# jeuneS2/csolve

Measured on AMD Instinct MI355X. Metric: constraint propagations/sec + nodes/sec, queens-N, 1/2/4/8 MI355X, higher is better.
Workload: dtype int32

## Files before the change

csolve_amd/csrc/cs_capi.hip:

```cpp
#include <hip/hip_runtime.h>
#include <chrono>

#include <dlfcn.h>
#include <stdarg.h>
#include <stdio.h>
#include <stdlib.h>
#include <string.h>

#include <mutex>

#include "../../include/csolve_gpu.h"
#include "cs_kernels.hip.h"
#include "cs_shave.hip.h"
#include "cs_step.hip.h"
#include "cs_dive.hip.h"
#include "cs_walk.hip.h"
#include "cs_chain.hip.h"
#include "cs_internal.h"

static thread_local char g_err[512] = "";

static int set_err(int code, const char *fmt, ...) {
  va_list ap;
  va_start(ap, fmt);
// ... 884 lines not shown
  if ((rc = lds_limit((size_t)h->n_vars * sizeof(cs_val) + 16, (const void *)cs_eval_root))) return rc;
  if ((rc = lds_limit((size_t)h->n_vars * sizeof(cs_val) + 16, (const void *)cs_eval_clauses))) return rc;
  if ((rc = plan_kernel(&m->plan.traced, (const void *)cs_propagate_events<true, false, true>, m->slice * CS_WAVES_PER_BLOCK,
                        CS_WAVES_PER_BLOCK)))
    return rc;
  const int per = (m->img->n_clauses + CS_WAVE - 1) / CS_WAVE;
  m->plan.rounds_cpl = m->img->n_clauses <= 0 || per > 8 ? 0 : (per <= 1 ? 1 : (per <= 2 ? 2 : (per <= 4 ? 4 : 8)));
  if (m->plan.rounds_cpl) {
#define CS_PICK6(CPL)                                                                              \
  m->plan.rounds.fn = m->has_tree_adj ? (const void *)cs_propagate_clause_rounds<CPL, true>         \
                                      : (const void *)cs_propagate_clause_rounds<CPL, false>
    switch (m->plan.rounds_cpl) {
    case 1: CS_PICK6(1); break;
    case 2: CS_PICK6(2); break;
    case 4: CS_PICK6(4); break;
    default: CS_PICK6(8); break;
    }
#undef CS_PICK6
    m->plan.rounds.lds = ((((size_t)h->n_vars * sizeof(cs_val) + 16 + 15) & ~(size_t)15)) * CS_WAVES_PER_BLOCK;
    m->plan.rounds.waves = CS_WAVES_PER_BLOCK;
    m->plan.rounds.per_cu = 8;
    if (m->plan.rounds.lds <= CS_CU_LDS) {
      for (int family = 0; family < WALK_FAMILIES; family++) {
        cs_planned *k = &m->plan.walk[family];
        if ((rc = plan_kernel(k, walk_kernel(family, m->plan.rounds_cpl, m->has_tree_adj), m->plan.rounds.lds, CS_WAVES_PER_BLOCK)))
          return rc;
        int occ = 0;
        if (hipOccupancyMaxActiveBlocksPerMultiprocessor(&occ, k->fn, CS_BLOCK, k->lds) == hipSuccess && occ >= 1 && occ < k->per_cu)
          k->per_cu = occ;
        if (k->per_cu < 1) k->per_cu = 1;
      }
      if ((rc = upload(h->dom, (size_t)h->n_vars * sizeof(cs_val), (int **)&m->d_walk_root))) return rc;
    }
  }
  m->plan.max_width = 2;
  for (int32_t v = 0; v < h->n_vars; v++) {
    const int64_t w = (int64_t)h->dom[v].hi - (int64_t)h->dom[v].lo + 1;
    if (w > m->plan.max_width) m->plan.max_width = w > 0x7fffffff ? 0x7fffffff : (int)w;
  }
  return CSGPU_OK;
}

static int plan_lds_resident(csgpu_model *m) {
  const cs_model *h = m->host;
  if (m->img->packed_width == 0) return CSGPU_OK;
  const size_t off_bytes = (((size_t)h->n_vars * 2 * sizeof(int)) + 15) & ~(size_t)15;
  const size_t adj_bytes = (((size_t)m->img->n_adj * (size_t)m->img->packed_width) + 15) & ~(size_t)15;
  const size_t lds_slice = ((size_t)h->n_vars * sizeof(cs_val) + (2 * (size_t)m->tab.n_words + 1) * sizeof(unsigned) + 15) & ~(size_t)15;
  m->lds_adj_global = 0;
  int waves_max = 16, waves = 0;
  size_t bytes = 0;
  { const char *e = getenv("CSGPU_K2_WAVES"); if (e != NULL && atoi(e) >= 4 && atoi(e) <= 16) waves_max = atoi(e); }
  for (int w = waves_max; w >= 4; w--) {
    const size_t need = off_bytes + adj_bytes + (size_t)w * lds_slice;
    if (need <= CS_CU_LDS) {
      waves = w;
      bytes = need;
      break;
    }
  }
  const char *force = getenv("CSGPU_K2_ADJ");
  const int want_global = force != NULL && force[0] == 'g';
  if (want_global && 8 * lds_slice <= CS_CU_LDS) {
    m->lds_adj_global = 1;
    waves = 8;
    bytes = 8 * lds_slice;
  }
  { const char *e = getenv("CSGPU_K2_CSZ"); m->k2_csz = e != NULL && atoi(e) >= 1 && atoi(e) <= CS_CHUNK ? atoi(e) : 0; }
  if (!waves) return CSGPU_OK;
  int rc;
  if ((rc = upload(m->img->adj_packed, (size_t)m->img->n_adj * (size_t)m->img->packed_width, (int **)&m->d_adj_packed)))
    return rc;
  if ((rc = plan_kernel(&m->plan.lds, ne_lds_kernel(m->img->packed_width, h->n_vars, m->lds_adj_global), bytes, waves)))
    return rc;
  if (m->plan.lds.per_cu < 1) m->plan.lds.per_cu = 1;
  return CSGPU_OK;
}

static int64_t widest_root_domain(const csgpu_model *m) {
  const cs_model *h = m->host;
  int64_t width = 1;
  for (int32_t v = 0; v < h->n_vars; v++) {
    const int64_t w = (int64_t)h->dom[v].hi - (int64_t)h->dom[v].lo + 1;
    if (w > width) width = w;
  }
  return width;
}

static int forbidden_sets_shape(const csgpu_model *m, int *fw_out, size_t *lds_out) {
  const cs_model *h = m->host;
  if (m->img->sym_width == 0 || m->not_root) return 0;
  const int64_t width = widest_root_domain(m);
  const int fw = width <= 64 ? 1 : (width <= 128 ? 2 : (width <= 256 ? 4 : 0));
  if (!fw) return 0;
  const size_t n_words = ((size_t)h->n_vars + 31) / 32;
  const size_t off_bytes = (((size_t)h->n_vars * 2 * sizeof(int)) + 15) & ~(size_t)15;
  const size_t base_bytes = (((size_t)h->n_vars * sizeof(int)) + 15) & ~(size_t)15;
  const size_t adj_bytes = (((size_t)m->img->sym_n_adj * (size_t)m->img->sym_width) + 15) & ~(size_t)15;
  const size_t sl = ((size_t)h->n_vars * sizeof(cs_val) + (size_t)h->n_vars * fw * 8 + (2 * n_words + 2) * sizeof(unsigned) + 15) &
                    ~(size_t)15;
  int waves = 16;
  for (; waves >= 1; waves--)
    if (off_bytes + base_bytes + adj_bytes + (size_t)waves * sl <= CS_CU_LDS) break;
  if (waves < 1) return 0;
  *fw_out = fw;
  *lds_out = off_bytes + base_bytes + adj_bytes + (size_t)waves * sl;
  return waves;
}

static int plan_forbidden_sets(csgpu_model *m) {
  const cs_model *h = m->host;
  int fw = 0;
  size_t lds = 0;
  const int waves = forbidden_sets_shape(m, &fw, &lds);
  if (!waves) return CSGPU_OK;
  m->fb_words = fw;
  int *lo = (int *)malloc((size_t)(h->n_vars ? h->n_vars : 1) * sizeof(int));
  for (int32_t v = 0; v < h->n_vars; v++) lo[v] = h->dom[v].lo;
  int rc = upload(lo, (size_t)h->n_vars * sizeof(int), &m->d_root_lo);
  free(lo);
  if (rc) return rc;
  if ((rc = upload(m->img->sym_off, ((size_t)h->n_vars + 1) * sizeof(int), &m->d_sym_off))) return rc;
  if ((rc = upload(m->img->sym_packed, (size_t)m->img->sym_n_adj * (size_t)m->img->sym_width, (int **)&m->d_sym_packed)))
    return rc;
  if ((rc = plan_kernel(&m->plan.bitset, ne_bitset_kernel(m->img->sym_width, fw, h->n_vars), lds, waves))) return rc;
  if (m->plan.bitset.per_cu < 1) m->plan.bitset.per_cu = 1;
  return CSGPU_OK;
}

static int dense_table_waves(const csgpu_model *m, size_t *bytes_out) {
  if (m->img->dense_width == 0) return 0;
  const size_t bytes = (size_t)m->host->n_vars * m->img->dense_slots * m->img->dense_cols * m->img->dense_width;
  int best = 0, waves = 0;
  for (int w = 4; w <= 16; w <<= 1)
    if (resident_per_cu(bytes, w) * w > best) { best = resident_per_cu(bytes, w) * w; waves = w; }
  *bytes_out = bytes;
  return waves;
}

static int plan_dense_table(csgpu_model *m) {
  const cs_model *h = m->host;
  if (!m->fb_words) return CSGPU_OK;
  const int n = h->n_vars, width = m->img->dense_width, slots = m->img->dense_slots;
  size_t bytes = 0;
  const int waves = dense_table_waves(m, &bytes);
  if (!waves) return CSGPU_OK;
  m->dense_bytes = bytes;
  int rc;
  if ((rc = upload(m->img->dense_tab, bytes, (int **)&m->d_dense_tab))) return rc;
  for (int variant = 0; variant < 4; variant++)
    if ((rc = plan_kernel(&m->plan.regs[variant], ne_regs_kernel(width, m->fb_words, n, variant & 1, variant >> 1), bytes, waves)))
      return rc;
  m->plan.full = n == cs_dense_strides(n) * CS_WAVE;
  if ((rc = plan_kernel(&m->plan.shave, ne_shave_kernel(width, n, slots, m->plan.full), bytes, waves))) return rc;
  const size_t table = (bytes + 15) & ~(size_t)15;
  if (table + (size_t)waves * 32 <= CS_CU_LDS &&
      (rc = plan_kernel(&m->plan.step_shave, step_shave_kernel(width, n, slots, m->plan.full), table + (size_t)waves * 32, waves)))
    return rc;
  if (table + CS_SHAVE_TRACE_LDS * 16 <= CS_CU_LDS) {
    if ((rc = plan_kernel(&m->plan.shave_trace, ne_shave_trace_kernel(width, n, slots), table + CS_SHAVE_TRACE_LDS * 16, waves)))
      return rc;
    m->plan.server = m->plan.shave_trace;
    m->plan.server.fn = shave_server_kernel(width, n, slots);
  }
  const int64_t widest = widest_root_domain(m);
  for (int family = 0; family < MANY_FAMILIES; family++) {
    const int by_allowed = MANY_BY_ALLOWED(family);
    if (by_allowed && widest > CS_DIVE_ALLOWED_WIDTH) continue;
    if ((rc = plan_kernel(&m->plan.dive[family], dive_kernel(family, width, n, widest <= 32 ? 1 : 4), table, waves))) return rc;
  }
  {
    int *hi = (int *)malloc((size_t)n * sizeof(int));
    if (hi == NULL) return set_err(CSGPU_E_ARG, "out of memory");
    for (int32_t v = 0; v < n; v++) hi[v] = h->dom[v].hi;
    rc = upload(hi, (size_t)n * sizeof(int), &m->d_root_hi);
    free(hi);
    if (rc) return rc;
  }
  HIP_TRY(hipMalloc((void **)&m->d_tickets, (size_t)CS_TICKET_SLOTS * CS_TICKET_SLOT_WORDS * sizeof(unsigned)));
  HIP_TRY(hipMemset(m->d_tickets, 0, (size_t)CS_TICKET_SLOTS * CS_TICKET_SLOT_WORDS * sizeof(unsigned)));
  m->ticket_slots = CS_TICKET_SLOTS;
  m->shave_static = getenv("CSGPU_SHAVE_STATIC") != NULL;
  return CSGPU_OK;
}

static int plan_packed(csgpu_model *m) {
  const cs_model *h = m->host;
  if (m->plan.shave.fn == NULL) return CSGPU_OK;
  const int n = h->n_vars, s3 = m->img->dense_slots == 3;
  m->packed_nw = 1;
  for (int32_t v = 0; v < n; v++)
    if ((int64_t)h->dom[v].hi - (int64_t)h->dom[v].lo + 1 > 32) m->packed_nw = 2;
  m->packed_bias = 0;
  for (int32_t v = 0; v < n; v++)
    if (h->dom[v].lo - m->img->dense_dmin > m->packed_bias) m->packed_bias = h->dom[v].lo - m->img->dense_dmin;
  m->plan.packed_nodes = packed_nodes_per_wave(m->fb_words, n, m->img->dense_width);
  if (!m->plan.packed_nodes) return CSGPU_OK;
  const size_t bytes = m->dense_bytes;
  int rc;
  if ((rc = plan_kernel(&m->plan.packed, ne_packed_kernel(n, m->packed_nw, s3), 2 * bytes, m->plan.regs[0].waves))) return rc;
  m->plan.packed.per_cu = m->plan.regs[0].per_cu;
  const size_t per_row = (size_t)m->img->dense_slots * m->img->dense_cols, total = (size_t)n * per_row;
  uint16_t *rel = (uint16_t *)malloc(total * sizeof(uint16_t));
  const uint8_t *src = (const uint8_t *)m->img->dense_tab;
  for (size_t i = 0; i < total; i++) {
    const int32_t u = (int32_t)(i / per_row);
    rel[i] = src[i] == 0xffu ? (uint16_t)0xffffu : (uint16_t)((int)src[i] - (h->dom[u].lo - m->img->dense_dmin) + m->packed_bias);
  }
  rc = upload(rel, total * sizeof(uint16_t), (int **)&m->d_packed_tab);
  free(rel);
  if (rc) return rc;
  if (step_packed_lds(m, 16) <= 80u * 1024u &&
      ((rc = plan_kernel(&m->plan.step_packed, step_packed_kernel(n, m->packed_nw, s3), step_packed_lds(m, 16), 16)) ||
       (rc = plan_kernel(&m->plan.step_import, step_import_kernel(n, m->packed_nw, s3), (2 * bytes + 15) & ~(size_t)15, 4))))
    return rc;
  m->step_chunk_max = 128;
  { const char *e = getenv("CSGPU_STEP_CHUNK_MAX"); if (e != NULL && atoi(e) > 0) m->step_chunk_max = atoi(e); }
  return CSGPU_OK;
}

static int stage_single_node(csgpu_model *m) {
  int dev = 0;
  hipDeviceProp_t prop;
  HIP_TRY(hipGetDevice(&dev));
  HIP_TRY(hipGetDeviceProperties(&prop, dev));
  m->n_cus = prop.multiProcessorCount;
  const size_t nbytes = (size_t)(m->host->n_vars ? m->host->n_vars : 1) * sizeof(cs_val);
  const size_t part = (nbytes + 63) & ~(size_t)63;
  unsigned char *d = NULL;
  HIP_TRY(hipHostMalloc((void **)&m->h_one, 2 * part + 128, hipHostMallocMapped));
  HIP_TRY(hipHostGetDevicePointer((void **)&d, m->h_one, 0));
  m->d_one_in = (cs_val *)d;
  m->d_one_node = (cs_node_in *)(d + part);
  m->d_one_res = (cs_node_out *)(d + part + 64);
  m->d_one_out = (cs_val *)(d + part + 128);
  return CSGPU_OK;
}

extern "C" int csgpu_model_finalize(csgpu_model *m) {
  if (m == NULL) return set_err(CSGPU_E_ARG, "null argument");
  free_device(m);
  int rc;
  if ((rc = csgpu_model_build_tables(m)) || (rc = drop_entailed_clauses(m)) || (rc = plan_general(m)) ||
      (rc = plan_lds_resident(m)) || (rc = plan_forbidden_sets(m)) || (rc = plan_dense_table(m)) || (rc = plan_packed(m)) ||
      (rc = stage_single_node(m)))
    return rc;
  m->plan.step_kind = m->plan.step_packed.fn != NULL ? 1
                      : (m->plan.step_shave.fn != NULL && m->host->n_vars <= 256 && m->plan.max_width <= 256 ? 2 : 0);
  m->finalized = 1;
  return CSGPU_OK;
}

static int kernel_qualifies(const csgpu_model *m, int which) {
  if (!m->finalized) return 0;
  switch (which) {
  case 1: return 1;
  case 2: return m->plan.lds.fn != NULL;
  case 3: return m->plan.bitset.fn != NULL;
  case 4: return m->plan.regs[0].fn != NULL;
  case 5: return m->plan.packed.fn != NULL;
  case 6: return m->plan.rounds.fn != NULL;
  case 7: return m->plan.shave.fn != NULL;
  default: return 0;
  }
}

extern "C" int csgpu_model_set_kernel(csgpu_model *m, int which) {
  static const char *const kernel_name[8] = {
    NULL, NULL, "the LDS-resident kernel", "the forbidden-set kernel", "the register-resident forbidden-set kernel",
    "the several-nodes-per-wave kernel (at most 32 variables, 64 values)", "the clause-resident kernel (at most 512 clauses)",
    "the interval-only shaving kernel (dense pair table in LDS)" };
  if (m == NULL || which < 0 || which > 7) return set_err(CSGPU_E_ARG, "bad argument");
  if (which >= 2) {
    if (!m->finalized) return set_err(CSGPU_E_STATE, "model is not finalized");
    if (!kernel_qualifies(m, which)) return set_err(CSGPU_E_LIMIT, "model does not qualify for %s", kernel_name[which]);
  }
  m->kernel_choice = which;
  return CSGPU_OK;
}

extern "C" int csgpu_model_qualifies(const csgpu_model *m, int which) { return m != NULL && kernel_qualifies(m, which); }

extern "C" int csgpu_internal_plan_symbol(const csgpu_model *m, int family, char *buf, size_t len) {
  if (m == NULL || buf == NULL || len == 0) return set_err(CSGPU_E_ARG, "null argument");
  if (!m->finalized) return set_err(CSGPU_E_STATE, "model is not finalized");
  const cs_kernel_plan *p = &m->plan;
  const cs_planned *fam[] = { &p->events, &p->traced, &p->rounds, &p->lds, &p->bitset, &p->regs[0], &p->regs[1],
                              &p->regs[2], &p->regs[3], &p->packed, &p->shave, &p->shave_trace, &p->server,
                              &p->step_shave, &p->step_packed, &p->step_import };
  if (family < 0 || family >= (int)(sizeof fam / sizeof fam[0])) return set_err(CSGPU_E_ARG, "no plan family %d", family);
  buf[0] = '\0';
  const void *fn = fam[family]->fn;
  if (fn == NULL) return CSGPU_OK;
  Dl_info info;
  if (dladdr(fn, &info) == 0 || info.dli_sname == NULL || info.dli_saddr != fn)
    return set_err(CSGPU_E_STATE, "plan family %d: the kernel handle has no dynamic symbol", family);
  if (strlen(info.dli_sname) >= len) return set_err(CSGPU_E_LIMIT, "plan family %d: symbol longer than the buffer", family);
  strcpy(buf, info.dli_sname);
  return CSGPU_OK;
}

static int many_symbol(const csgpu_model *m, const cs_planned *k, const char *name, char *buf, size_t len) {
  if (m == NULL || buf == NULL || len == 0) return set_err(CSGPU_E_ARG, "null argument");
  if (!m->finalized) return set_err(CSGPU_E_STATE, "model is not finalized");
  buf[0] = '\0';
  const void *fn = k->fn;
  if (fn == NULL) return CSGPU_OK;
  Dl_info info;
// ... 1931 lines not shown
```

csolve_amd/csrc/cs_shave.hip.h:

```cpp
#ifndef CS_SHAVE_HIP_H
#define CS_SHAVE_HIP_H

#include "cs_kernels.hip.h"

#ifdef CS_SHAVE_TIMELINE
__device__ unsigned long long cs_shave_tl[3 * 65536];
#endif

__device__ __forceinline__ unsigned long long cs_bitset0(unsigned long long m, int i) {
  asm("s_bitset0_b64 %0, %1" : "+s"(m) : "s"(i));
  return m;
}

__device__ __forceinline__ void cs_shift_if_eq(int &lo, int &hi, int f) {
  unsigned long long c;
  asm("v_cmp_eq_u32 vcc, %0, %3\n\t"
      "v_cmp_eq_u32 %2, %1, %3\n\t"
      "v_addc_co_u32 %0, vcc, 0, %0, vcc\n\t"
      "v_subb_co_u32 %1, %2, %1, 0, %2"
      : "+v"(lo), "+v"(hi), "=&s"(c) : "v"(f) : "vcc");
}
__device__ __forceinline__ void cs_shift_if_eq3(int &lo, int &hi, int f0, int f1, int f2) {
  unsigned long long c;
  asm("v_cmp_eq_u32 vcc, %0, %3\n\t"
      "v_cmp_eq_u32 %2, %1, %3\n\t"
      "v_addc_co_u32 %0, vcc, 0, %0, vcc\n\t"
      "v_subb_co_u32 %1, %2, %1, 0, %2\n\t"
      "v_cmp_eq_u32 vcc, %0, %4\n\t"
      "v_cmp_eq_u32 %2, %1, %4\n\t"
      "v_addc_co_u32 %0, vcc, 0, %0, vcc\n\t"
      "v_subb_co_u32 %1, %2, %1, 0, %2\n\t"
      "v_cmp_eq_u32 vcc, %0, %5\n\t"
      "v_cmp_eq_u32 %2, %1, %5\n\t"
      "v_addc_co_u32 %0, vcc, 0, %0, vcc\n\t"
      "v_subb_co_u32 %1, %2, %1, 0, %2"
      : "+v"(lo), "+v"(hi), "=&s"(c) : "v"(f0), "v"(f1), "v"(f2) : "vcc");
}

__device__ __forceinline__ void cs_lanes_ne2(unsigned long long &m0, int a, int b, unsigned long long &m1, int c, int d) {
  asm("v_cmp_ne_u32 %0, %2, %3\n\tv_cmp_ne_u32 %1, %4, %5" : "=&s"(m0), "=s"(m1) : "v"(a), "v"(b), "v"(c), "v"(d));
}

__device__ __forceinline__ void cs_popc64x2(int &c0, unsigned long long m0, int &c1, unsigned long long m1) {
  asm("s_bcnt1_i32_b64 %0, %2\n\ts_bcnt1_i32_b64 %1, %3" : "=&s"(c0), "=s"(c1) : "s"(m0), "s"(m1) : "scc");
}

template <int L>
__device__ __forceinline__ int cs_writelane(int v, int x) {
  x = __builtin_amdgcn_readfirstlane(x);
  asm("v_writelane_b32 %0, %1, %2" : "+v"(v) : "s"(x), "n"(L));
  return v;
}

__device__ __forceinline__ int cs_writelane_at(int lane, int v, int x) {
  switch (lane) {
  case 0: return cs_writelane<0>(v, x);
  case 1: return cs_writelane<1>(v, x);
  case 2: return cs_writelane<2>(v, x);
  default: return cs_writelane<3>(v, x);
  }
}

#define CS_SHAVE_TRACE_LDS 2048u
#define CS_SHAVE_CHUNK 2
#define CS_SHAVE_SHARDS 64
#define CS_SHAVE_TICKET_STRIDE 16

template <typename E, int R, int SL, bool TRACE>
struct cs_shave_core {
  typedef unsigned long long u64;
  static constexpr int W = CS_WAVE * R;
  const E *s_tab;
  int slots, lane;
  int kb[R], deg[R], b0[R];
  u64 livemask[R];
  int4 *s_trace;
  unsigned tcount;

  __device__ __forceinline__ void trace_lanes(u64 mask, int r2, int kind, int value, int cause) {
    if (mask == 0ull) return;
    const unsigned at = tcount + __builtin_amdgcn_mbcnt_hi((unsigned)(mask >> 32), __builtin_amdgcn_mbcnt_lo((unsigned)mask, 0u));
    if (__builtin_amdgcn_inverse_ballot_w64(mask) && at < CS_SHAVE_TRACE_LDS)
      s_trace[at] = make_int4(lane + r2 * CS_WAVE, kind, value + b0[r2], cause);
    tcount += (unsigned)__builtin_popcountll(mask);
  }

  __device__ __forceinline__ void push_var(int r, int ul, int cd, int (&rlo)[R], int (&rhi)[R], u64 (&dl)[R], u64 (&dh)[R],
                                           int &revisions) {
    revisions += __builtin_amdgcn_readlane(deg[r], ul);
    const E *row = s_tab + (size_t)(ul + r * CS_WAVE) * slots * W + lane;
    int plo[R], phi[R];
    if (TRACE) {
#pragma unroll
      for (int r2 = 0; r2 < R; r2++) { plo[r2] = rlo[r2]; phi[r2] = rhi[r2]; }
    }
    if (SL == 3) {
#pragma unroll
      for (int r2 = 0; r2 < R; r2++) {
        const int f0 = cd - (int)row[r2 * CS_WAVE];
        const int f1 = cd - (int)row[W + r2 * CS_WAVE];
        const int f2 = cd - (int)row[2 * W + r2 * CS_WAVE];
        cs_shift_if_eq3(rlo[r2], rhi[r2], f0, f1, f2);
      }
    } else if (SL != 0) {
#pragma unroll
      for (int k = 0; k < (SL ? SL : 1); k++) {
#pragma unroll
        for (int r2 = 0; r2 < R; r2++) cs_shift_if_eq(rlo[r2], rhi[r2], cd - (int)row[k * W + r2 * CS_WAVE]);
      }
    } else {
      for (int k = 0; k < slots; k++) {
#pragma unroll
        for (int r2 = 0; r2 < R; r2++) cs_shift_if_eq(rlo[r2], rhi[r2], cd - (int)row[k * W + r2 * CS_WAVE]);
      }
    }
    if (TRACE) {
#pragma unroll
      for (int r2 = 0; r2 < R; r2++) {
        const u64 ml = __ballot(rlo[r2] != plo[r2]), mh = __ballot(rhi[r2] != phi[r2]);
        dl[r2] |= ml;
        dh[r2] |= mh;
        trace_lanes(ml, r2, 0, rlo[r2], ul + r * CS_WAVE);
        trace_lanes(mh, r2, 1, rhi[r2], ul + r * CS_WAVE);
      }
    }
  }

  __device__ __forceinline__ void push_phase(const u64 (&who)[R], int (&rlo)[R], int (&rhi)[R], u64 (&pushed)[R], u64 (&dl)[R],
                                             u64 (&dh)[R], int &revisions) {
    int cdv[R], plo[R], phi[R];
#pragma unroll
    for (int r = 0; r < R; r++) { cdv[r] = rlo[r] + kb[r]; plo[r] = rlo[r]; phi[r] = rhi[r]; }
#pragma unroll
    for (int r = 0; r < R; r++) {
      u64 bits = who[r];
      pushed[r] |= bits;
      while (bits != 0ull) {
        const int ul = __builtin_ctzll(bits);
        bits = cs_bitset0(bits, ul);
        push_var(r, ul, __builtin_amdgcn_readlane(cdv[r], ul), rlo, rhi, dl, dh, revisions);
      }
    }
    if (!TRACE) {
#pragma unroll
      for (int r = 0; r < R; r++) {
        u64 ml, mh;
        cs_lanes_ne2(ml, rlo[r], plo[r], mh, rhi[r], phi[r]);
        dl[r] |= ml;
        dh[r] |= mh;
      }
    }
  }

  __device__ __forceinline__ int settle(const int (&rlo)[R], const int (&rhi)[R], u64 (&val)[R]) const {
    int bad = -1;
#pragma unroll
    for (int r = R - 1; r >= 0; r--) {
      const u64 c = __ballot(rlo[r] > rhi[r]);
      if (c != 0ull) bad = __builtin_ctzll(c) + r * CS_WAVE;
      val[r] = __ballot(rlo[r] == rhi[r]) & livemask[r];
    }
    return __builtin_amdgcn_readfirstlane(bad);
  }

  __device__ __forceinline__ bool sweep_pays(const u64 (&dl)[R], const u64 (&dh)[R], const u64 (&val)[R]) const {
    int n_dirty = 0, n_val = 0;
#pragma unroll
    for (int r = 0; r < R; r++) {
      int d, v;
      cs_popc64x2(d, dl[r] | dh[r], v, val[r]);
      n_dirty += d;
      n_val += v;
    }
    return n_dirty > n_val;
  }

  template <bool CAUSE>
  __device__ __forceinline__ u64 forbidders(const E *row, const int (&e)[SL ? SL : 1][R], int ckw, const int (&rlo)[R],
                                            const u64 (&val)[R], int &cause) const {
    u64 hit = 0ull;
    if (SL != 0) {
#pragma unroll
      for (int r2 = 0; r2 < R; r2++) {
        const int t = ckw - rlo[r2];
        u64 h = 0ull;
#pragma unroll
        for (int k = 0; k < (SL ? SL : 1); k++) h |= __ballot(e[k][r2] == t);
        hit |= h & val[r2];
        if (TRACE && CAUSE && cause < 0 && (h & val[r2]) != 0ull) cause = __builtin_ctzll(h & val[r2]) + r2 * CS_WAVE;
      }
    } else {
      for (int k = 0; k < slots; k++) {
#pragma unroll
        for (int r2 = 0; r2 < R; r2++) {
          const u64 h = __ballot((int)row[k * W + r2 * CS_WAVE] == ckw - rlo[r2]) & val[r2];
          hit |= h;
          if (TRACE && CAUSE && cause < 0 && h != 0ull) cause = __builtin_ctzll(h) + r2 * CS_WAVE;
        }
      }
    }
    return hit;
  }

  template <int SIDE>
  __device__ __forceinline__ void verify_side(int (&rlo)[R], int (&rhi)[R], u64 (&dirty)[R], u64 (&val)[R], int &revisions,
                                              int &fail_v) {
#pragma unroll
    for (int r = 0; r < R; r++) {
      u64 bits = dirty[r];
      dirty[r] = 0ull;
      while (bits != 0ull) {
        const int wl = __builtin_ctzll(bits);
        bits = cs_bitset0(bits, wl);
        int cand = __builtin_amdgcn_readlane(SIDE == 0 ? rlo[r] : rhi[r], wl);
        const int ckw = cand + __builtin_amdgcn_readlane(kb[r], wl);
        revisions += __builtin_amdgcn_readlane(deg[r], wl);
        const E *row = s_tab + (size_t)(wl + r * CS_WAVE) * slots * W + lane;
        int e[SL ? SL : 1][R];
        if (SL != 0) {
#pragma unroll
          for (int k = 0; k < (SL ? SL : 1); k++)
#pragma unroll
            for (int r2 = 0; r2 < R; r2++) e[k][r2] = (int)row[k * W + r2 * CS_WAVE];
        }
        int cause = -1;
        if (forbidders<true>(row, e, ckw, rlo, val, cause) != 0ull) {
          const int other = __builtin_amdgcn_readlane(SIDE == 0 ? rhi[r] : rlo[r], wl);
          int step = 0;
          bool on;
          do {
            step++;
            on = SIDE == 0 ? cand + step <= other : cand - step >= other;
            if (on) on = forbidders<false>(row, e, ckw + (SIDE == 0 ? step : -step), rlo, val, cause) != 0ull;
          } while (on);
          cand += SIDE == 0 ? step : -step;
          if (lane == wl) { if (SIDE == 0) rlo[r] = cand; else rhi[r] = cand; }
          if (TRACE) trace_lanes(1ull << wl, r, SIDE, cand, cause);
          if (SIDE == 0 ? cand > other : cand < other) fail_v = wl + r * CS_WAVE;
          if (cand == other) val[r] |= 1ull << wl;
        }
      }
    }
  }

  __device__ __forceinline__ int round(int (&rlo)[R], int (&rhi)[R], u64 (&pushed)[R], u64 (&push)[R], u64 (&dl)[R],
                                       u64 (&dh)[R], u64 (&val)[R], int &revisions, bool &more) {
    more = false;
    push_phase(push, rlo, rhi, pushed, dl, dh, revisions);
    int fail_v = settle(rlo, rhi, val);
    if (fail_v < 0) {
      if (sweep_pays(dl, dh, val)) {
        bool again;
        do {
          u64 who[R];
#pragma unroll
          for (int r = 0; r < R; r++) { who[r] = val[r]; dl[r] = 0ull; dh[r] = 0ull; }
          push_phase(who, rlo, rhi, pushed, dl, dh, revisions);
          fail_v = settle(rlo, rhi, val);
          again = fail_v < 0;
          if (again) again = sweep_pays(dl, dh, val);
        } while (again);
      }
      if (fail_v < 0) {
        verify_side<0>(rlo, rhi, dl, val, revisions, fail_v);
        verify_side<1>(rlo, rhi, dh, val, revisions, fail_v);
        fail_v = __builtin_amdgcn_readfirstlane(fail_v);
        if (fail_v < 0) {
          u64 any_push = 0ull;
#pragma unroll
          for (int r = 0; r < R; r++) {
            push[r] = val[r] & ~pushed[r];
            any_push |= push[r];
          }
          more = any_push != 0ull;
        }
      }
    }
    return fail_v;
  }

  __device__ __forceinline__ int fixpoint(int (&rlo)[R], int (&rhi)[R], u64 (&pushed)[R], u64 (&push)[R], u64 (&dl)[R],
                                          u64 (&dh)[R], u64 (&val)[R], int &rounds, int &revisions) {
    bool more;
    int fail_v;
    if (TRACE) {
      do {
        fail_v = round(rlo, rhi, pushed, push, dl, dh, val, revisions, more);
        if (more) {
          if (rounds == 0) __builtin_amdgcn_s_setprio(3);
          rounds++;
        }
      } while (more);
      return fail_v;
    }
    fail_v = round(rlo, rhi, pushed, push, dl, dh, val, revisions, more);
    if (more) {
      if (rounds == 0) __builtin_amdgcn_s_setprio(3);
      do {
        rounds++;
        fail_v = round(rlo, rhi, pushed, push, dl, dh, val, revisions, more);
      } while (more);
    }
    return fail_v;
  }
};

template <typename E, int R, int SL, bool FULL, bool TRACE = false>
__global__ __launch_bounds__(1024, (R <= 2 ? 8 : 4)) void cs_propagate_ne_shave(
    int n, const E *__restrict__ tab_g, int slots, int dmin, const int *__restrict__ root_lo,
    const int *__restrict__ sym_off, const cs_val *__restrict__ states_in, const cs_node_in *__restrict__ nodes,
    cs_val *__restrict__ states_out, cs_node_out *__restrict__ results, long long batch,
    const unsigned long long *__restrict__ batch_dev, int csz , unsigned *tickets,
    int4 *__restrict__ trace, unsigned *__restrict__ trace_n, unsigned trace_cap) {
  extern __shared__ __attribute__((aligned(16))) unsigned char cs_lds[];
  typedef unsigned long long u64;
  constexpr int W = CS_WAVE * R;
  constexpr int D = R == 1 && !TRACE ? 2 * CS_SHAVE_CHUNK : CS_SHAVE_CHUNK;
  if (batch_dev != nullptr && (long long)*batch_dev < batch) batch = (long long)*batch_dev;
  const int nbatch = __builtin_amdgcn_readfirstlane((int)batch);
  const int lane = threadIdx.x & (CS_WAVE - 1);
  const int wave_in_block = __builtin_amdgcn_readfirstlane(threadIdx.x >> 6);
  const int waves_per_block = blockDim.x >> 6;
  const int chunks = (nbatch + csz - 1) / csz;
  const int nsh = (int)gridDim.x < CS_SHAVE_SHARDS ? (int)gridDim.x : CS_SHAVE_SHARDS;
  const int shard = (int)(blockIdx.x % nsh);
  const int count_x = chunks > shard ? (chunks - 1 - shard) / nsh + 1 : 0;
  const int waves_x = (((int)gridDim.x - 1 - shard) / nsh + 1) * waves_per_block;
  const int wave_local = (int)(blockIdx.x / nsh) * waves_per_block + wave_in_block;
  const bool dynamic = tickets != nullptr && count_x > waves_x;
  if ((int)(blockIdx.x / nsh) * waves_per_block >= count_x) return;
  if (SL != 0) slots = SL;
  const E *s_tab = (const E *)cs_lds;
  int4 *s_trace = (int4 *)(cs_lds + ((((size_t)n * slots * W * sizeof(E)) + 15) & ~(size_t)15));
  {
    const int vecs = (int)(((size_t)n * slots * W * sizeof(E)) / 16);
    const uint4 *src = (const uint4 *)tab_g;
    uint4 *dst = (uint4 *)cs_lds;
    for (int i = threadIdx.x; i < vecs; i += blockDim.x) dst[i] = src[i];
  }
#ifdef CS_SHAVE_TIMELINE
  const unsigned long long tl_start = __builtin_amdgcn_s_memrealtime();
  unsigned long long tl_nodes = 0;
#endif
  __syncthreads();
  if (wave_local >= count_x) return;

  int b0[R], kb[R], deg[R], vcl[R];
  bool live[R];
#pragma unroll
  for (int r = 0; r < R; r++) {
    const int v = lane + r * CS_WAVE;
    live[r] = FULL || v < n;
    vcl[r] = live[r] ? v : n - 1;
    b0[r] = live[r] ? root_lo[vcl[r]] : 0;
    kb[r] = b0[r] - dmin;
    deg[r] = live[r] ? sym_off[vcl[r] + 1] - sym_off[vcl[r]] : 0;
  }
  u64 livemask[R];
#pragma unroll
  for (int r = 0; r < R; r++) livemask[r] = FULL ? ~0ull : __ballot(live[r]);
  cs_shave_core<E, R, SL, TRACE> C;
  C.s_tab = s_tab; C.slots = slots; C.lane = lane; C.s_trace = s_trace; C.tcount = 0u;
#pragma unroll
  for (int r = 0; r < R; r++) { C.kb[r] = kb[r]; C.deg[r] = deg[r]; C.b0[r] = b0[r]; C.livemask[r] = livemask[r]; }
  unsigned *my_ticket = tickets + (size_t)shard * CS_SHAVE_TICKET_STRIDE;

  auto load_rec = [&](int i) {
    cs_node_in rec;
    rec.var = -1; rec.lo = 0; rec.hi = 0; rec.parent = 0;
    const int node = (i * nsh + shard) * csz + lane;
    if (lane < csz && node < nbatch) rec = nodes[node];
    return rec;
  };
  auto next_index = [&](int i_prev, unsigned tk_v) -> int {
    if (!dynamic) return i_prev + waves_x;
    const int t = __builtin_amdgcn_readfirstlane((int)tk_v);
    if (t == count_x - 1 && lane == 0) __hip_atomic_store(my_ticket, 0u, __ATOMIC_RELAXED, __HIP_MEMORY_SCOPE_AGENT);
    return waves_x + t;
  };
  auto draw = [&]() -> unsigned {
    unsigned tk_v = 0;
    if (lane == 0) tk_v = __hip_atomic_fetch_add(my_ticket, 1u, __ATOMIC_RELAXED, __HIP_MEMORY_SCOPE_AGENT);
    return tk_v;
  };

  int i_cur = wave_local;
  cs_node_in rec_cur = load_rec(i_cur);
  unsigned tk = dynamic ? draw() : 0u;
  cs_val pd[D][R];
#pragma unroll
  for (int d = 0; d < D; d++) {
    const size_t prow = (size_t)__builtin_amdgcn_readlane(rec_cur.parent, d) * n;
#pragma unroll
    for (int r = 0; r < R; r++) pd[d][r] = states_in[prow + vcl[r]];
  }
  int i_next = next_index(i_cur, tk);
  int have_next = i_next < count_x;
  cs_node_in rec_next = load_rec(have_next ? i_next : i_cur);

  for (;;) {
    i_cur = __builtin_amdgcn_readfirstlane(i_cur);
    i_next = __builtin_amdgcn_readfirstlane(i_next);
    have_next = i_next < count_x;
    if (have_next && dynamic) tk = draw();
    cs_val pn[D][R];
#pragma unroll
    for (int d = 0; d < D; d++)
#pragma unroll
      for (int r = 0; r < R; r++) pn[d][r] = pd[d][r];
    if (have_next) {
#pragma unroll
      for (int d = 0; d < D; d++) {
        const size_t prow = (size_t)__builtin_amdgcn_readlane(rec_next.parent, d) * n;
#pragma unroll
        for (int r = 0; r < R; r++) pn[d][r] = states_in[prow + vcl[r]];
      }
    }
    const int base = (i_cur * nsh + shard) * csz;
    const int cnt = nbatch - base < csz ? nbatch - base : csz;
#ifdef CS_SHAVE_TIMELINE
    tl_nodes += cnt;
#endif
    cs_node_out my_result;
    my_result.status = 0; my_result.props = 0; my_result.revisions = 0; my_result.rounds = 0;
#pragma unroll
    for (int dd = 0; dd < D; dd++) {
      const int j = dd;
      if (j >= cnt) continue;
      const int nvar = __builtin_amdgcn_readlane(rec_cur.var, j);
      const int nlo = __builtin_amdgcn_readlane(rec_cur.lo, j), nhi = __builtin_amdgcn_readlane(rec_cur.hi, j);
      int rlo[R], rhi[R];
#pragma unroll
      for (int r = 0; r < R; r++) {
        rlo[r] = live[r] ? pd[dd][r].lo - b0[r] : 0;
        rhi[r] = live[r] ? pd[dd][r].hi - b0[r] : 0;
      }

      u64 pushed[R], push[R], dl[R], dh[R];
#pragma unroll
      for (int r = 0; r < R; r++) {
        pushed[r] = nvar < 0 ? ~livemask[r] : __ballot(rlo[r] == rhi[r]);
        dl[r] = 0ull; dh[r] = 0ull;
      }
#pragma unroll
      for (int r = 0; r < R; r++) {
        if (nvar >= 0 && (nvar >> 6) == r) {
          const u64 bit = 1ull << (nvar & 63);
          if (lane == (nvar & 63)) { rlo[r] = nlo - b0[r]; rhi[r] = nhi - b0[r]; }
          pushed[r] &= ~bit;
          if (nlo != nhi) { dl[r] |= bit; dh[r] |= bit; }
        }
      }
      int lo0[R], hi0[R];
#pragma unroll
      for (int r = 0; r < R; r++) { lo0[r] = rlo[r]; hi0[r] = rhi[r]; }
      u64 val[R];
#pragma unroll
      for (int r = 0; r < R; r++) {
        val[r] = __ballot(rlo[r] == rhi[r]) & livemask[r];
        push[r] = val[r] & ~pushed[r];
      }

      C.tcount = 0u;
      int rounds = 0, revisions = 0;
      const int fail_var = C.fixpoint(rlo, rhi, pushed, push, dl, dh, val, rounds, revisions);
      const int failed = fail_var >= 0;
      if (TRACE) {
        const unsigned keep = C.tcount < CS_SHAVE_TRACE_LDS ? C.tcount : CS_SHAVE_TRACE_LDS;
        for (unsigned i = lane; i < keep && i < trace_cap; i += CS_WAVE) trace[i] = s_trace[i];
        if (lane == 0) *trace_n = C.tcount;
      }
      if (rounds != 0) __builtin_amdgcn_s_setprio(0);

      int open_vars = 0, shaved = 0;
#pragma unroll
      for (int r = 0; r < R; r++) {
        open_vars += __popcll(__ballot(rlo[r] != rhi[r]));
        shaved += (rlo[r] - lo0[r]) + (hi0[r] - rhi[r]);
      }
      const int props = cs_wave_sum(shaved);
      const size_t orow = (size_t)(unsigned)(base + j) * (unsigned)n;
#ifndef CS_SHAVE_STORE_FAILED
#define CS_SHAVE_STORE_FAILED 0
#endif
      if (FULL && (CS_SHAVE_STORE_FAILED || !failed)) {
#pragma unroll
        for (int r = 0; r < R; r++) states_out[orow + lane + r * CS_WAVE] = cs_interval(rlo[r] + b0[r], rhi[r] + b0[r]);
      } else if (!FULL && !failed) {
#pragma unroll
        for (int r = 0; r < R; r++)
          if (live[r]) states_out[orow + lane + r * CS_WAVE] = cs_interval(rlo[r] + b0[r], rhi[r] + b0[r]);
      }
      my_result.status = cs_writelane_at(dd, my_result.status, failed ? -1 : open_vars);
      my_result.props = cs_writelane_at(dd, my_result.props, props);
      my_result.revisions = cs_writelane_at(dd, my_result.revisions, revisions);
      my_result.rounds = cs_writelane_at(dd, my_result.rounds, failed ? fail_var : rounds);
    }
    if (lane < cnt) results[base + lane] = my_result;

    if (!have_next) break;
    const int i_nn = next_index(i_next, tk);
    const int have_nn = i_nn < count_x;
    i_cur = i_next;
    rec_cur = rec_next;
#pragma unroll
    for (int d = 0; d < D; d++)
#pragma unroll
      for (int r = 0; r < R; r++) pd[d][r] = pn[d][r];
    rec_next = load_rec(have_nn ? i_nn : i_next);
    i_next = i_nn;
    have_next = have_nn;
  }
#ifdef CS_SHAVE_TIMELINE
  if (lane == 0) {
    const size_t w = ((size_t)blockIdx.x * (blockDim.x >> 6) + (threadIdx.x >> 6)) % 65536;
    cs_shave_tl[3 * w] = tl_start;
    cs_shave_tl[3 * w + 1] = __builtin_amdgcn_s_memrealtime();
    cs_shave_tl[3 * w + 2] = tl_nodes;
  }
#endif
}

struct cs_mailbox_head {
  unsigned req_seq; unsigned pad0[15];
  unsigned ack_seq; unsigned alive; unsigned pad1[14];
  unsigned stop; unsigned pad2[15];
  cs_node_in node; unsigned want_trace; unsigned pad3[11];
  cs_node_out result; unsigned trace_n; unsigned pad4[11];
};

template <typename E, int R, int SL>
__global__ __launch_bounds__(1024) void cs_shave_server(int n, const E *__restrict__ tab_g, int slots, int dmin,
                                                        const int *__restrict__ root_lo, const int *__restrict__ sym_off,
                                                        cs_mailbox_head *box, unsigned long long *state_in ,
                                                        unsigned long long *state_out , int4 *trace ,
                                                        unsigned trace_cap, unsigned long long idle_ticks) {
  extern __shared__ __attribute__((aligned(16))) unsigned char cs_lds[];
  typedef unsigned long long u64;
  constexpr int W = CS_WAVE * R;
  const int lane = threadIdx.x & (CS_WAVE - 1);
  if (SL != 0) slots = SL;
  {
    const int vecs = (int)(((size_t)n * slots * W * sizeof(E)) / 16);
    const uint4 *src = (const uint4 *)tab_g;
    uint4 *dst = (uint4 *)cs_lds;
    for (int i = threadIdx.x; i < vecs; i += blockDim.x) dst[i] = src[i];
  }
  int4 *s_trace = (int4 *)(cs_lds + ((((size_t)n * slots * W * sizeof(E)) + 15) & ~(size_t)15));
  __syncthreads();
  if (threadIdx.x >= CS_WAVE) return;

  cs_shave_core<E, R, SL, true> C;
  C.s_tab = (const E *)cs_lds; C.slots = slots; C.lane = lane; C.s_trace = s_trace; C.tcount = 0u;
  int b0[R];
  bool live[R];
#pragma unroll
  for (int r = 0; r < R; r++) {
    const int v = lane + r * CS_WAVE;
    live[r] = v < n;
    const int vc = live[r] ? v : n - 1;
    b0[r] = live[r] ? root_lo[vc] : 0;
    C.b0[r] = b0[r];
    C.kb[r] = b0[r] - dmin;
    C.deg[r] = live[r] ? sym_off[vc + 1] - sym_off[vc] : 0;
    C.livemask[r] = __ballot(live[r]);
  }
  unsigned last = __hip_atomic_load(&box->ack_seq, __ATOMIC_RELAXED, __HIP_MEMORY_SCOPE_SYSTEM);
  if (lane == 0) __hip_atomic_store(&box->alive, 1u, __ATOMIC_RELEASE, __HIP_MEMORY_SCOPE_SYSTEM);
  u64 idle_since = __builtin_amdgcn_s_memrealtime();
  for (;;) {
    const unsigned seq = __hip_atomic_load(&box->req_seq, __ATOMIC_ACQUIRE, __HIP_MEMORY_SCOPE_SYSTEM);
    if (seq == last) {
      if (__hip_atomic_load(&box->stop, __ATOMIC_RELAXED, __HIP_MEMORY_SCOPE_SYSTEM) != 0u) break;
      if (__builtin_amdgcn_s_memrealtime() - idle_since > idle_ticks) break;
      __builtin_amdgcn_s_sleep(2);
      continue;
    }
    const int nvar = (int)__hip_atomic_load((unsigned *)&box->node.var, __ATOMIC_RELAXED, __HIP_MEMORY_SCOPE_SYSTEM);
    const int nlo = (int)__hip_atomic_load((unsigned *)&box->node.lo, __ATOMIC_RELAXED, __HIP_MEMORY_SCOPE_SYSTEM);
    const int nhi = (int)__hip_atomic_load((unsigned *)&box->node.hi, __ATOMIC_RELAXED, __HIP_MEMORY_SCOPE_SYSTEM);
    const unsigned want_trace = __hip_atomic_load(&box->want_trace, __ATOMIC_RELAXED, __HIP_MEMORY_SCOPE_SYSTEM);
    int rlo[R], rhi[R];
#pragma unroll
    for (int r = 0; r < R; r++) {
      const int v = lane + r * CS_WAVE;
      const u64 e = __hip_atomic_load(&state_in[live[r] ? v : n - 1], __ATOMIC_RELAXED, __HIP_MEMORY_SCOPE_SYSTEM);
      rlo[r] = live[r] ? (int)(unsigned)e - b0[r] : 0;
      rhi[r] = live[r] ? (int)(unsigned)(e >> 32) - b0[r] : 0;
    }
    u64 pushed[R], push[R], dl[R], dh[R], val[R];
#pragma unroll
    for (int r = 0; r < R; r++) {
      pushed[r] = nvar < 0 ? ~C.livemask[r] : __ballot(rlo[r] == rhi[r]);
      dl[r] = 0ull; dh[r] = 0ull;
    }
#pragma unroll
    for (int r = 0; r < R; r++) {
      if (nvar >= 0 && (nvar >> 6) == r) {
        const u64 bit = 1ull << (nvar & 63);
        if (lane == (nvar & 63)) { rlo[r] = nlo - b0[r]; rhi[r] = nhi - b0[r]; }
        pushed[r] &= ~bit;
        if (nlo != nhi) { dl[r] |= bit; dh[r] |= bit; }
      }
    }
    int lo0[R], hi0[R];
#pragma unroll
    for (int r = 0; r < R; r++) {
      lo0[r] = rlo[r]; hi0[r] = rhi[r];
      val[r] = __ballot(rlo[r] == rhi[r]) & C.livemask[r];
      push[r] = val[r] & ~pushed[r];
    }
    C.tcount = 0u;
    int rounds = 0, revisions = 0;
    const int fail_var = C.fixpoint(rlo, rhi, pushed, push, dl, dh, val, rounds, revisions);
    if (rounds != 0) __builtin_amdgcn_s_setprio(0);
    const int failed = fail_var >= 0;
    int open_vars = 0, shaved = 0;
#pragma unroll
    for (int r = 0; r < R; r++) {
      open_vars += __popcll(__ballot(rlo[r] != rhi[r]));
      shaved += (rlo[r] - lo0[r]) + (hi0[r] - rhi[r]);
    }
    const int props = cs_wave_sum(shaved);
    if (!failed) {
#pragma unroll
      for (int r = 0; r < R; r++)
        if (live[r]) {
          const u64 e = (u64)(unsigned)(rlo[r] + b0[r]) | ((u64)(unsigned)(rhi[r] + b0[r]) << 32);
          __hip_atomic_store(&state_out[lane + r * CS_WAVE], e, __ATOMIC_RELAXED, __HIP_MEMORY_SCOPE_SYSTEM);
        }
    }
    if (want_trace != 0u) {
      const unsigned keep = C.tcount < CS_SHAVE_TRACE_LDS ? C.tcount : CS_SHAVE_TRACE_LDS;
      for (unsigned i = lane; i < keep && i < trace_cap; i += CS_WAVE) trace[i] = s_trace[i];
    }
    if (lane == 0) {
      box->result.status = failed ? -1 : open_vars;
      box->result.props = props;
      box->result.revisions = revisions;
      box->result.rounds = failed ? fail_var : rounds;
      box->trace_n = C.tcount;
    }
    __builtin_amdgcn_fence(__ATOMIC_RELEASE, "");
    if (lane == 0) __hip_atomic_store(&box->ack_seq, seq, __ATOMIC_RELEASE, __HIP_MEMORY_SCOPE_SYSTEM);
    last = seq;
    idle_since = __builtin_amdgcn_s_memrealtime();
  }
  if (lane == 0) __hip_atomic_store(&box->alive, 0u, __ATOMIC_RELEASE, __HIP_MEMORY_SCOPE_SYSTEM);
}

#endif
```

Baseline: 21.25 billion.

## Use 16-byte per-lane row loads/stores via LDS restaging in single-stride shave kernel

For the full, single-stride (n=64) shave kernel, parent state rows are fetched as 16-byte chunks covering two rows per load and transposed through a per-wave LDS scratch area. Output rows are likewise paired in LDS and written with 16-byte stores, masked per half for failed nodes. The host planner now reserves per-wave LDS for this scratch and picks a waves-per-block count that maximizes resident waves. The aim is fewer, wider global memory transactions, at the cost of extra LDS traffic, wave barriers and possibly lower occupancy.

```diff
diff --git a/csolve_amd/csrc/cs_capi.hip b/csolve_amd/csrc/cs_capi.hip
--- a/csolve_amd/csrc/cs_capi.hip
+++ b/csolve_amd/csrc/cs_capi.hip
@@ -1060,8 +1060,20 @@
     if ((rc = plan_kernel(&m->plan.regs[variant], ne_regs_kernel(width, m->fb_words, n, variant & 1, variant >> 1), bytes, waves)))
       return rc;
   m->plan.full = n == cs_dense_strides(n) * CS_WAVE;
-  if ((rc = plan_kernel(&m->plan.shave, ne_shave_kernel(width, n, slots, m->plan.full), bytes, waves))) return rc;
   const size_t table = (bytes + 15) & ~(size_t)15;
+  {
+    size_t shave_lds = bytes;
+    int shave_waves = waves;
+    if (m->plan.full && cs_dense_strides(n) == 1) {
+      int best = 0;
+      for (int w = 4; w <= 16; w <<= 1) {
+        const size_t lds = table + (size_t)w * CS_SHAVE_WIDE_LDS;
+        if (lds <= CS_CU_LDS && resident_per_cu(lds, w) * w >= best) { best = resident_per_cu(lds, w) * w; shave_waves = w; shave_lds = lds; }
+      }
+      if (!best) shave_waves = 0;
+    }
+    if (shave_waves && (rc = plan_kernel(&m->plan.shave, ne_shave_kernel(width, n, slots, m->plan.full), shave_lds, shave_waves))) return rc;
+  }
   if (table + (size_t)waves * 32 <= CS_CU_LDS &&
       (rc = plan_kernel(&m->plan.step_shave, step_shave_kernel(width, n, slots, m->plan.full), table + (size_t)waves * 32, waves)))
     return rc;
diff --git a/csolve_amd/csrc/cs_shave.hip.h b/csolve_amd/csrc/cs_shave.hip.h
--- a/csolve_amd/csrc/cs_shave.hip.h
+++ b/csolve_amd/csrc/cs_shave.hip.h
@@ -65,6 +65,9 @@
 #define CS_SHAVE_CHUNK 2
 #define CS_SHAVE_SHARDS 64
 #define CS_SHAVE_TICKET_STRIDE 16
+#define CS_SHAVE_WIDE_LDS 3072u
+
+struct __attribute__((aligned(4))) cs_row16 { unsigned x, y, z, w; };
 
 template <typename E, int R, int SL, bool TRACE>
 struct cs_shave_core {
@@ -316,6 +319,7 @@
   typedef unsigned long long u64;
   constexpr int W = CS_WAVE * R;
   constexpr int D = R == 1 && !TRACE ? 2 * CS_SHAVE_CHUNK : CS_SHAVE_CHUNK;
+  constexpr bool WIDE = R == 1 && FULL && !TRACE;
   if (batch_dev != nullptr && (long long)*batch_dev < batch) batch = (long long)*batch_dev;
   const int nbatch = __builtin_amdgcn_readfirstlane((int)batch);
   const int lane = threadIdx.x & (CS_WAVE - 1);
@@ -344,6 +348,7 @@
 #endif
   __syncthreads();
   if (wave_local >= count_x) return;
+  uint4 *s_rows = (uint4 *)(cs_lds + ((((size_t)n * slots * W * sizeof(E)) + 15) & ~(size_t)15)) + wave_in_block * (CS_SHAVE_WIDE_LDS / 16);
 
   int b0[R], kb[R], deg[R], vcl[R];
   bool live[R];
@@ -384,15 +389,44 @@
     return tk_v;
   };
 
+  const int low_half = (lane >> 5) - 1;
+  auto fetch_rows = [&](const cs_node_in &rec, cs_row16 (&pw)[D / 2]) {
+#pragma unroll
+    for (int p = 0; p < D / 2; p++) {
+      const int pa = __builtin_amdgcn_readlane(rec.parent, 2 * p), pb = __builtin_amdgcn_readlane(rec.parent, 2 * p + 1);
+      const int par = pb ^ ((pa ^ pb) & low_half);
+      pw[p] = *(const cs_row16 *)((const unsigned char *)states_in + (size_t)par * 512 + (lane & 31) * 16);
+    }
+  };
+  auto restage = [&](const cs_row16 (&pw)[D / 2], cs_val (&rows)[D][R]) {
+    __builtin_amdgcn_fence(__ATOMIC_ACQ_REL, "wavefront");
+    __builtin_amdgcn_wave_barrier();
+#pragma unroll
+    for (int p = 0; p < D / 2; p++) s_rows[p * CS_WAVE + lane] = make_uint4(pw[p].x, pw[p].y, pw[p].z, pw[p].w);
+    __builtin_amdgcn_fence(__ATOMIC_ACQ_REL, "wavefront");
+    __builtin_amdgcn_wave_barrier();
+#pragma unroll
+    for (int d = 0; d < D; d++) {
+      const uint2 v = ((const uint2 *)s_rows)[d * CS_WAVE + lane];
+      rows[d][0] = cs_interval((int)v.x, (int)v.y);
+    }
+  };
+
   int i_cur = wave_local;
   cs_node_in rec_cur = load_rec(i_cur);
   unsigned tk = dynamic ? draw() : 0u;
   cs_val pd[D][R];
-#pragma unroll
-  for (int d = 0; d < D; d++) {
-    const size_t prow = (size_t)__builtin_amdgcn_readlane(rec_cur.parent, d) * n;
-#pragma unroll
-    for (int r = 0; r < R; r++) pd[d][r] = states_in[prow + vcl[r]];
+  if (WIDE) {
+    cs_row16 pw[D / 2];
+    fetch_rows(rec_cur, pw);
+    restage(pw, pd);
+  } else {
+#pragma unroll
+    for (int d = 0; d < D; d++) {
+      const size_t prow = (size_t)__builtin_amdgcn_readlane(rec_cur.parent, d) * n;
+#pragma unroll
+      for (int r = 0; r < R; r++) pd[d][r] = states_in[prow + vcl[r]];
+    }
   }
   int i_next = next_index(i_cur, tk);
   int have_next = i_next < count_x;
@@ -404,16 +438,21 @@
     have_next = i_next < count_x;
     if (have_next && dynamic) tk = draw();
     cs_val pn[D][R];
-#pragma unroll
-    for (int d = 0; d < D; d++)
-#pragma unroll
-      for (int r = 0; r < R; r++) pn[d][r] = pd[d][r];
-    if (have_next) {
-#pragma unroll
-      for (int d = 0; d < D; d++) {
-        const size_t prow = (size_t)__builtin_amdgcn_readlane(rec_next.parent, d) * n;
-#pragma unroll
-        for (int r = 0; r < R; r++) pn[d][r] = states_in[prow + vcl[r]];
+    cs_row16 pw[D / 2];
+    if (WIDE) {
+      if (have_next) fetch_rows(rec_next, pw);
+    } else {
+#pragma unroll
+      for (int d = 0; d < D; d++)
+#pragma unroll
+        for (int r = 0; r < R; r++) pn[d][r] = pd[d][r];
+      if (have_next) {
+#pragma unroll
+        for (int d = 0; d < D; d++) {
+          const size_t prow = (size_t)__builtin_amdgcn_readlane(rec_next.parent, d) * n;
+#pragma unroll
+          for (int r = 0; r < R; r++) pn[d][r] = states_in[prow + vcl[r]];
+        }
       }
     }
     const int base = (i_cur * nsh + shard) * csz;
@@ -423,6 +462,7 @@
 #endif
     cs_node_out my_result;
     my_result.status = 0; my_result.props = 0; my_result.revisions = 0; my_result.rounds = 0;
+    bool even_ok = false;
 #pragma unroll
     for (int dd = 0; dd < D; dd++) {
       const int j = dd;
@@ -483,7 +523,24 @@
 #ifndef CS_SHAVE_STORE_FAILED
 #define CS_SHAVE_STORE_FAILED 0
 #endif
-      if (FULL && (CS_SHAVE_STORE_FAILED || !failed)) {
+      if (WIDE && !CS_SHAVE_STORE_FAILED) {
+        __builtin_amdgcn_fence(__ATOMIC_ACQ_REL, "wavefront");
+        __builtin_amdgcn_wave_barrier();
+        ((uint2 *)(s_rows + 2 * CS_WAVE))[(dd & 1) * CS_WAVE + lane] = make_uint2((unsigned)(rlo[0] + b0[0]), (unsigned)(rhi[0] + b0[0]));
+        if (!(dd & 1)) even_ok = !failed;
+        if ((dd & 1) || dd + 1 >= cnt) {
+          const u64 halves = (even_ok ? 0x00000000ffffffffull : 0ull) | ((dd & 1) && !failed ? 0xffffffff00000000ull : 0ull);
+          if (halves != 0ull) {
+            __builtin_amdgcn_fence(__ATOMIC_ACQ_REL, "wavefront");
+            __builtin_amdgcn_wave_barrier();
+            const uint4 o = s_rows[2 * CS_WAVE + lane];
+            cs_row16 o16;
+            o16.x = o.x; o16.y = o.y; o16.z = o.z; o16.w = o.w;
+            if (__builtin_amdgcn_inverse_ballot_w64(halves))
+              *(cs_row16 *)((unsigned char *)states_out + (size_t)(unsigned)(base + (dd & ~1)) * 512 + lane * 16) = o16;
+          }
+        }
+      } else if (FULL && (CS_SHAVE_STORE_FAILED || !failed)) {
 #pragma unroll
         for (int r = 0; r < R; r++) states_out[orow + lane + r * CS_WAVE] = cs_interval(rlo[r] + b0[r], rhi[r] + b0[r]);
       } else if (!FULL && !failed) {
@@ -503,10 +560,14 @@
     const int have_nn = i_nn < count_x;
     i_cur = i_next;
     rec_cur = rec_next;
-#pragma unroll
-    for (int d = 0; d < D; d++)
-#pragma unroll
-      for (int r = 0; r < R; r++) pd[d][r] = pn[d][r];
+    if (WIDE) {
+      restage(pw, pd);
+    } else {
+#pragma unroll
+      for (int d = 0; d < D; d++)
+#pragma unroll
+        for (int r = 0; r < R; r++) pd[d][r] = pn[d][r];
+    }
     rec_next = load_rec(have_nn ? i_nn : i_next);
     i_next = i_nn;
     have_next = have_nn;
```

Result: slower. 20.90 billion (-1.7%).
